# TritonDataCenter/containerpilot

Hardware: NVIDIA H100
Metric: events/sec through Bus.Publish (deliveries/s = 32-byte records landed in subscriber mailboxes) (higher is better)
Workload: dtype u8

## Files before the change

### containerpilot_b200/csrc/cpbus.cu

```cuda
#include "cpbus_kernels.cuh"

#include <algorithm>
#include <chrono>
#include <cstdio>
#include <cstdlib>
#include <cstring>
#include <deque>
#include <map>
#include <mutex>
#include <new>
#include <string>
#include <thread>
#include <unordered_map>
#include <vector>

using namespace cpbus_dev;

namespace {

thread_local char g_cuda_err[256] = "";

#define CK(call)                                                                                   \
  do {                                                                                             \
    cudaError_t e_ = (call);                                                                       \
// ... 561 lines not shown
  static bool done[64] = {};
  static std::mutex mu;
  std::lock_guard<std::mutex> g(mu);
  if (done[b->device & 63]) return CPBUS_OK;
  int rc;
  if ((rc = preload_round_fanouts<CPBUS_STORE_V4>()) || (rc = preload_round_fanouts<CPBUS_STORE_V8>()) ||
      (rc = preload_round_fanouts<CPBUS_STORE_BULK>()))
    return rc;
  cudaFuncAttributes a;
  CK(cudaFuncGetAttributes(&a, stream_round_decide_kernel));
  CK(cudaFuncGetAttributes(&a, stream_round_admit_kernel));
  CK(cudaFuncGetAttributes(&a, stream_round_agree_kernel));
  CK(cudaFuncGetAttributes(&a, consume_all_kernel));
  CK(cudaFuncGetAttributes(&a, digest_fold_kernel));
  CK(cudaFuncGetAttributes(&a, blockers_scan_kernel));
  CK(cudaFuncGetAttributes(&a, lagging_scan_kernel));
  done[b->device & 63] = true;
  return CPBUS_OK;
}

struct StreamArgs {
  const StreamHdr* hdr = nullptr; unsigned long long* ack = nullptr; unsigned long long seq = 0;
  const StreamHdr* next_hdr = nullptr;
  uint32_t off = 0; bool final = true;
  FollowRec* follow_rec = nullptr;
  bool follow_from_host = false;
  const RoundDev* round = nullptr;
};

struct LaunchOpts {
  int staged = 0;
  const cpbus_event* pf_src = nullptr;
  cpbus_event* pf_dst = nullptr;
  uint32_t pf_n = 0;
  bool batch_dep = false;
  bool account = false;
  const StreamArgs* stream = nullptr;
};

DevResultSlot* result_slot(const cpbus* b, unsigned long long seq) {
  return b->d_result + (size_t)(seq % kResultRing) * kResultSub;
}

void launched_to(cpbus* b, uint64_t w) {
  b->last_watermark = w;
  if (b->sparse) due_fire(b->due, b->h_timers, w, [](uint32_t, uint64_t, uint64_t) {});
}

int launch_fanout(cpbus* b, const cpbus_event* d_src, uint32_t n, uint64_t w, const LaunchOpts& o = {}) {
  const StreamArgs* sa = o.stream;
  if (b->n_next == 0 && !sa) return CPBUS_OK;
  if (n == 0 && b->n_timers == 0 && !sa) return CPBUS_OK;
  FanoutParams p{};
  p.batch = d_src; p.ring = b->d_ring; p.ctl = b->d_ctl; p.timers = b->d_timers; p.stats = b->d_stats; p.pow_table = b->d_pow; p.launch_seq = ++b->launch_seq;
  p.desc = b->d_desc + (p.launch_seq & 1) * ((fanout_desc_bytes(2048) + 255) & ~(size_t)255);
  p.desc_ready = b->d_desc_ready + (p.launch_seq & 1) * 16; p.w_now = w;
  p.result = result_slot(b, p.launch_seq); p.result_next = result_slot(b, p.launch_seq + 1);
  p.batch_local = b->d_batch_local; p.staged = (uint32_t)o.staged;
  p.err_word = b->d_err; p.acct = o.account ? b->d_acct : nullptr;
  p.pf_state = b->d_pf_state; p.pf_buf = b->d_pf_buf; p.pf_stride = b->B; p.spin_us = b->stream_spin_us;
  if (sa) {
    p.stream_hdr = sa->hdr; p.stream_ack = sa->ack; p.stream_seq = sa->seq; p.stream_next_hdr = sa->next_hdr;
    p.stream_off = sa->off; p.stream_final = sa->final ? 1u : 0u;
  }
  const bool follow = sa && sa->follow_rec, round = sa && sa->round;
  const int kind = round ? kLaunchRound : follow ? kLaunchFollow : kLaunchPlain;
  p.round = round ? sa->round : nullptr;
  if (follow) {
    p.follow_clock = b->d_follow_clock; p.follow_rec = sa->follow_rec; p.follow_window = max_window(b);
    p.follow_from_host = sa->follow_from_host ? 1u : 0u;
  }
  p.prefetch_src = o.pf_src; p.prefetch_dst = o.pf_dst; p.prefetch_n = o.pf_n;
  p.batch_dep = o.batch_dep ? 1u : 0u; p.n_ev = n;
  p.n_subs = b->n_next; p.ring_cap = b->R; p.K = b->K; p.sub_base = b->cfg.sub_id_base;
  p.use_digest = b->use_digest; p.lossless = b->lossless; p.timers_on = b->n_timers > 0 && b->K > 0;
  p.smem_cap = (n + 31u) & ~31u;
  const size_t hot_bytes = (size_t)b->n_next * (sizeof(SubCtl) + (p.timers_on ? b->K * sizeof(DevTimer) : 0));
  p.hints = b->hints >= 0 ? (uint32_t)b->hints : (hot_bytes <= (64u << 20) ? 1u : 0u);
  const uint32_t need = (b->n_next + kWarpsPerCta - 1) / kWarpsPerCta;
  uint32_t grid = b->cfg.grid_ctas ? std::max(1u, std::min(b->cfg.grid_ctas, need)) : 0u;
  int rc;
  const bool pairs_on = b->n_paired > 0 && b->d_pairs;
  p.pairs = pairs_on ? b->d_pairs : nullptr;
  size_t smem = fanout_smem_bytes(p.smem_cap) + (pairs_on ? kPairFilterBytes : 0);
  if (!pairs_on && !p.timers_on && b->n_filtered > 0) {
    if (b->order_dirty) { const int rc_order = rebuild_order(b); if (rc_order) return rc_order; }
    if (b->n_order) {
      const uint32_t scale = std::max(1u, (p.n_ev + 128u) / 256u);
      uint32_t spw = b->subs_per_warp ? std::min(32u, b->subs_per_warp)
                                      : std::max(4u, std::min(16u / scale, b->n_order / (20480u * scale)));
      p.order = b->d_order; p.n_order = b->n_order; p.spw = spw;
      const uint32_t warps = (b->n_order + spw - 1) / spw;
      grid = std::max(1u, (warps + kWarpsPerCta - 1) / kWarpsPerCta);
    }
  }
  if (pairs_on && !b->cfg.grid_ctas) {
    const uint32_t blocks = (b->n_next + 31u) / 32u;
    grid = std::max(1u, std::min((blocks + kWarpsPerCta - 1) / kWarpsPerCta, (uint32_t)b->sm_count * 16u));
  }
  if (!pairs_on && !p.order) {
    uint32_t spw = b->subs_per_warp;
    if (grid) spw = std::max(1u, (need + grid - 1) / grid);
    else if (!spw) {
      const uint32_t scale = std::max(1u, (p.n_ev + 128u) / 256u);
      const uint32_t cap = std::max(1u, 16u / scale);
      spw = std::max(1u, std::min(cap, (need + (uint32_t)b->sm_count * 7 * scale) / ((uint32_t)b->sm_count * 14 * scale)));
    }
    p.spw = spw;
    grid = std::max(1u, (need + spw - 1) / spw);
    const size_t off = fanout_stage_off(p.smem_cap);
    const size_t per_sub = sizeof(SubCtl) + (p.timers_on ? (size_t)b->K * sizeof(DevTimer) : 0);
    const size_t min_round = (size_t)kWarpsPerCta * per_sub;
    const size_t ctas = std::max<size_t>(1, std::min<size_t>(kCtasPerSm, b->smem_per_sm / (off + min_round + b->smem_reserved)));
    const size_t room = std::min<size_t>(kFanoutMaxSmem, b->smem_per_sm / ctas - b->smem_reserved) - off;
    p.stage_subs = std::max<uint32_t>(kWarpsPerCta, (uint32_t)std::min<size_t>((size_t)kWarpsPerCta * spw, room / per_sub) & ~7u);
    smem = off + p.stage_subs * per_sub;
  }
  const int variant = pairs_on ? (p.use_digest ? 7 : 6) : (p.timers_on ? 2 : 0) | (p.use_digest ? 1 : 0) | (p.order ? 4 : 0);
#define CPBUS_DISPATCH(ST)                                                                \
  switch (variant) {                                                                     \
    case 0: rc = launch_fanout_t<ST, false, false, false>(b, p, grid, smem, kind); break;      \
    case 1: rc = launch_fanout_t<ST, false, true, false>(b, p, grid, smem, kind); break;       \
    case 2: rc = launch_fanout_t<ST, true, false, false>(b, p, grid, smem, kind); break;       \
    case 3: rc = launch_fanout_t<ST, true, true, false>(b, p, grid, smem, kind); break;        \
    case 4: rc = launch_fanout_t<ST, false, false, true>(b, p, grid, smem, kind); break;       \
    case 5: rc = launch_fanout_t<ST, false, true, true>(b, p, grid, smem, kind); break;        \
    case 6: rc = launch_fanout_t<ST, true, false, false, true>(b, p, grid, smem, kind); break; \
    default: rc = launch_fanout_t<ST, true, true, false, true>(b, p, grid, smem, kind); break; \
  }
  switch (b->store) {
    case CPBUS_STORE_V4: CPBUS_DISPATCH(CPBUS_STORE_V4); break;
    case CPBUS_STORE_BULK: CPBUS_DISPATCH(CPBUS_STORE_BULK); break;
    default: CPBUS_DISPATCH(CPBUS_STORE_V8); break;
  }
#undef CPBUS_DISPATCH
  if (rc) return rc;
  b->st.kernel_launches++;
  if (!round) b->st.batches++;
  if (sa) return CPBUS_OK;
  launched_to(b, w);
  if (o.account && n) dbg_mark_device_batch(b, p.launch_seq);
  return CPBUS_OK;
}

void timer_table(cpbus* b) {
  b->h_timers.resize((size_t)b->N * b->K);
  if (b->sparse) b->due.init(b->h_timers.size());
}

int stage_batch(cpbus* b, uint32_t n, cpbus_event** d_dst) {
  const uint32_t slot = b->dev_slot;
  *d_dst = b->d_stage + (size_t)slot * b->B;
  if (slot % cpbus::kDevEpoch == 0) CK(cudaEventSynchronize(b->epoch_done[slot / cpbus::kDevEpoch]));
  if (n) {
    CK(cudaMemcpyAsync(*d_dst, b->h_batch[b->cur], (size_t)n * sizeof(cpbus_event), cudaMemcpyHostToDevice, b->copy_stream));
    CK(cudaEventRecord(b->h2d_done[b->cur], b->copy_stream));
  }
  return CPBUS_OK;
}

int retire_slot(cpbus* b) {
  const uint32_t slot = b->dev_slot;
  if (slot % cpbus::kDevEpoch == cpbus::kDevEpoch - 1) CK(cudaEventRecord(b->epoch_done[slot / cpbus::kDevEpoch], b->stream));
  b->dev_slot = (slot + 1) % cpbus::kDevSlots;
  return CPBUS_OK;
}

int await_copy(cpbus* b, cudaEvent_t copied) {
  const auto t_spin = std::chrono::steady_clock::now();
  do {
    const cudaError_t q = cudaEventQuery(copied);
    if (q == cudaSuccess) return CPBUS_OK;
    if (q != cudaErrorNotReady) { CK(q); }
  } while (std::chrono::steady_clock::now() - t_spin < std::chrono::microseconds(30));
  CK(cudaStreamWaitEvent(b->stream, copied, 0));
  return CPBUS_OK;
}

int next_buffer(cpbus* b) {
  b->cur = (b->cur + 1) % cpbus::kStage;
  CK(cudaEventSynchronize(b->h2d_done[b->cur]));
  return CPBUS_OK;
}

size_t sparse_max(const cpbus* b) { return std::max<size_t>(32, b->n_next / 1024); }
size_t sparse_max_deliveries(const cpbus* b) { return std::max<size_t>(1024, b->n_next / 256); }

int plan_room(cpbus* b, size_t bytes) {
  if (bytes <= b->plan_bytes_cap) { CK(cudaEventSynchronize(b->plan_done)); return CPBUS_OK; }
  CK(cudaStreamSynchronize(b->stream)); CK(cudaStreamSynchronize(b->copy_stream));
  cudaFree(b->d_plan); cudaFreeHost(b->h_plan);
  b->d_plan = nullptr; b->h_plan = nullptr; b->plan_bytes_cap = 0;
  const size_t cap = std::max<size_t>(bytes, 64 << 10);
// ... 2447 lines not shown
```

### containerpilot_b200/csrc/cpbus_fanout_body.cuh

```cuda
  constexpr bool STAGED = !ORDERED && !PAIRS;
  extern __shared__ __align__(128) unsigned char smem[];
  const uint32_t cap = p.smem_cap;
  cpbus_event* s_batch = reinterpret_cast<cpbus_event*>(smem);
  uint64_t* s_rhash = reinterpret_cast<uint64_t*>(smem + (size_t)cap * 32);
  uint2* s_meta = reinterpret_cast<uint2*>(smem + (size_t)cap * 40);
  uint64_t* s_q = reinterpret_cast<uint64_t*>(smem + (size_t)cap * 48);
  uint32_t* s_dsum = reinterpret_cast<uint32_t*>(s_q + cap + 2);
  uint32_t* s_present = s_dsum + 40;
  uint64_t* s_pow = s_q + cap + 2 + 20 + (PAIRS ? kPairFilterWords / 2 : 0);
  BatchSummary* s_sum = reinterpret_cast<BatchSummary*>(s_pow + cap + 66);
  uint32_t* s_tick = reinterpret_cast<uint32_t*>(s_sum + 1);
  const uint4* s_ctl4 = reinterpret_cast<const uint4*>(smem + fanout_stage_off(cap));
  const uint4* s_tim4 = s_ctl4 + 2u * p.stage_subs;

  const int tid = threadIdx.x, lane = tid & 31, warp = tid >> 5;
  uint32_t n = FOLLOW ? 0u : p.n_ev;
  uint64_t w_follow = 0;
  unsigned long long round_ack = 0;

  if (p.batch_dep) asm volatile("griddepcontrol.wait;" ::: "memory");
  const bool stream = p.staged == 2u;
  const uint32_t pf_slot = stream ? (uint32_t)(p.stream_seq % kStreamPrefetch) : 0u;
  uint32_t pos = ORDERED ? (blockIdx.x * kWarpsPerCta + warp) * p.spw : 0u;
  uint32_t my_ids = 0;
  if (ORDERED && pos + lane < min(pos + p.spw, p.n_order)) my_ids = __ldg(p.order + pos + lane);
  if (tid == 0) {
    mbar_init(&s_sum->mbar, 1); mbar_init(&s_sum->mbar_desc, 1); mbar_init(&s_sum->mbar_state, 1);
    s_sum->acc_deliv = 0; s_sum->acc_ticks = 0; s_sum->acc_dig_lo = 0; s_sum->acc_dig_hi = 0;
    s_sum->stream_local = (stream && !p.lossless && p.stream_off == 0 && __ldcg(p.pf_state + pf_slot) == p.stream_seq) ? 1u : 0u;
    s_sum->own_desc = blockIdx.x == 0 ? 1u : 0u; s_sum->abort_launch = 0;
  }
  __syncthreads();
  const bool stream_local = stream && s_sum->stream_local;
  const bool staged = FOLLOW || (p.staged && !stream_local);
  const cpbus_event* batch_src = stream_local ? p.pf_buf + (size_t)pf_slot * p.pf_stride : p.batch;
  if (tid == 0) {
    const uint32_t pow_bytes = ((cap + 65u) * 8u + 15u) & ~15u;
    const bool direct = n && !staged;
    mbar_expect_tx(&s_sum->mbar, (direct ? n * 32u : 0u) + pow_bytes);
    if (direct) bulk_g2s(s_batch, batch_src, n * 32u, &s_sum->mbar);
    bulk_g2s(s_pow, p.pow_table, pow_bytes, &s_sum->mbar);
  }

  const bool keep = p.hints & 1u;

  const uint32_t desc_bytes = 24u * cap + 16u + 160u + (PAIRS ? kPairFilterBytes : 0u);
  uint4* s_desc = reinterpret_cast<uint4*>(s_rhash);
  uint4* g_desc = reinterpret_cast<uint4*>(p.desc);
  constexpr unsigned long long kAbortBit = 1ull << 63;
  if (blockIdx.x != 0) {
    if (tid == 0) {
      unsigned long long seen = 0;
      if (!(p.hints & 2u)) {
        unsigned long long t0, t1;
        asm volatile("mov.u64 %0, %%globaltimer;" : "=l"(t0));
        const unsigned long long budget = stream ? 4000000000ull : 200000ull;
        do {
          asm volatile("ld.acquire.gpu.global.u64 %0, [%1];" : "=l"(seen) : "l"(p.desc_ready) : "memory");
          if ((seen & ~kAbortBit) >= p.launch_seq) break;
          asm volatile("mov.u64 %0, %%globaltimer;" : "=l"(t1));
        } while (t1 - t0 < budget);
      }
      if ((seen & ~kAbortBit) < p.launch_seq) s_sum->own_desc = 1u;
      else {
        const bool ab = (seen & kAbortBit) != 0;
        s_sum->abort_launch = ab ? 1u : 0u;
        asm volatile("fence.proxy.async;" ::: "memory");
        mbar_expect_tx(&s_sum->mbar_desc, desc_bytes);
        bulk_g2s(s_desc, g_desc, desc_bytes, &s_sum->mbar_desc);
        const uint32_t n_copy = FOLLOW ? (ab ? 0u : *reinterpret_cast<const volatile uint32_t*>(p.desc + 24u * cap + 16u + 4u * kFollowN)) : n;
        if (staged && n_copy && !ab) {
          mbar_wait(&s_sum->mbar, 0);
          mbar_expect_tx(&s_sum->mbar, n_copy * 32u);
          bulk_g2s(s_batch, p.batch_local, n_copy * 32u, &s_sum->mbar);
        }
      }
    }
    __syncthreads();
  }
  const bool own_desc = s_sum->own_desc != 0;
  const bool lead = blockIdx.x == 0;
  if (own_desc) {
    if (lead && tid < kResultSub * 4) reinterpret_cast<unsigned long long*>(p.result_next)[tid] = 0ull;
    if (tid < 40) s_dsum[tid] = 0;
    if constexpr (ROUND) {
      __syncthreads();
      if (tid == 0) {
        const volatile RoundDev* rd = p.round;
        if (!rd->go) s_sum->abort_launch = 1u;
        else {
          const unsigned long long w = rd->w;
          s_dsum[kFollowN] = rd->m; s_dsum[kFollowWLo] = (uint32_t)w; s_dsum[kFollowWHi] = (uint32_t)(w >> 32);
          s_dsum[kRoundSrc] = rd->src;
          if (lead && rd->final) round_ack = rd->q;
        }
// ... 183 lines not shown
  const uint32_t K = p.K, J = K ? 32u / K : 32u;
  const uint32_t tk_slot = lane / J, tk_j = lane % J;
  const bool timers_on = TIMERS && p.timers_on && K;
  const uint32_t wstride = gridDim.x * kWarpsPerCta;
  uint32_t pos_end = (aborted || !ORDERED) ? 0u : min(pos + p.spw, p.n_order);
  const uint32_t pos_step = ORDERED ? 1u : kWarpsPerCta;
  const uint32_t pos0 = pos;
  uint32_t s = ORDERED ? __shfl_sync(0xffffffffu, my_ids, 0) : pos;
  if (!p.batch_dep) asm volatile("griddepcontrol.wait;" ::: "memory");
  asm volatile("griddepcontrol.launch_dependents;");
  const uint32_t rng_first = blockIdx.x * kWarpsPerCta * p.spw, rng_end = min(rng_first + kWarpsPerCta * p.spw, p.n_subs);
  auto stage_round = [&](uint32_t first) {
    if (!STAGED || tid != 0 || aborted || first >= rng_end) return;
    const uint32_t rn = min(p.stage_subs, rng_end - first);
    asm volatile("fence.proxy.async.shared::cta;" ::: "memory");
    const uint32_t tim_bytes = timers_on ? rn * K * (uint32_t)sizeof(DevTimer) : 0u;
    mbar_expect_tx(&s_sum->mbar_state, rn * (uint32_t)sizeof(SubCtl) + tim_bytes);
    bulk_g2s_hint(const_cast<uint4*>(s_ctl4), p.ctl + first, rn * (uint32_t)sizeof(SubCtl), &s_sum->mbar_state, keep);
    if (tim_bytes) bulk_g2s_hint(const_cast<uint4*>(s_tim4), p.timers + (size_t)first * K, tim_bytes, &s_sum->mbar_state, keep);
  };
  uint4 ca = make_uint4(0, 0, 0, 0), cb = ca, ta = ca;
  if (ORDERED && pos < pos_end) ld_sector(p.ctl + s, ca, cb, keep);
  const uint32_t present = s_dsum[0];
  const bool has_unicast = s_dsum[1] != 0;
  bool bulk_pending = false;
  uint32_t tri_blk = blockIdx.x * kWarpsPerCta + warp, tri_base = 0, tri_live = 0;
  uint4 tri_a = make_uint4(0, 0, 0, 0), tri_b = tri_a;
  uint32_t rnd_first = rng_first, rnd_phase = 0;
  for (;;) {
  if constexpr (STAGED) {
    if (aborted || rnd_first >= rng_end) break;
    stage_round(rnd_first);
    mbar_wait(&s_sum->mbar_state, rnd_phase);
    rnd_phase ^= 1u;
    pos = rnd_first + warp; pos_end = rnd_first + min(p.stage_subs, rng_end - rnd_first);
  }
  if constexpr (PAIRS) {
    bool exhausted = aborted;
    while (!tri_live && !exhausted) {
      tri_base = tri_blk * 32u;
      if (tri_base >= p.n_subs) { exhausted = true; break; }
      tri_blk += wstride;
      const uint32_t sl = tri_base + lane;
      bool live = false;
      tri_a = make_uint4(0, 0, 0, 0); tri_b = tri_a;
      if (sl < p.n_subs) ld_sector(p.ctl + sl, tri_a, tri_b, keep);
      const uint32_t ml = tri_b.z;
      if (ml & kActiveBit) {
        live = has_unicast || (ml & present) != 0;
        if (!live && timers_on) {
          const uint32_t nsl = min((ml >> kTimerHintShift) & 0xFu, K);
          for (uint32_t t = 0; t < nsl && !live; t++) {
            uint4 h;
            ld_half(p.timers + (size_t)sl * K + t, h, keep);
            const uint64_t due = ((uint64_t)h.y << 32) | h.x;
            live = due != kTimerIdle && due <= (FOLLOW ? w_follow : p.w_now);
          }
        }
        if (!live && (ml & kPairBit)) {
          const uint4* row = reinterpret_cast<const uint4*>(p.pairs + (size_t)sl * CPBUS_MAX_PAIRS);
          for (uint32_t q = 0; q < CPBUS_MAX_PAIRS / 2 && !live; q++) {
            const uint4 v = __ldg(row + q);
            if (v.x >= 32u) break;
            uint32_t h = pair_key_hash(v.x, v.y);
            live = ((s_present[(h & 32767u) >> 5] >> (h & 31u)) & (s_present[((h >> 15) & 32767u) >> 5] >> ((h >> 15) & 31u)) & 1u) != 0;
            if (live || v.z >= 32u) { if (!live) break; continue; }
            h = pair_key_hash(v.z, v.w);
            live = ((s_present[(h & 32767u) >> 5] >> (h & 31u)) & (s_present[((h >> 15) & 32767u) >> 5] >> ((h >> 15) & 31u)) & 1u) != 0;
          }
        }
      }
      tri_live = __ballot_sync(0xffffffffu, live);
    }
    if (exhausted) break;
    const uint32_t jl = (uint32_t)__ffs(tri_live) - 1u;
    tri_live &= tri_live - 1u;
    pos = tri_base + jl; pos_end = pos + 1u; s = pos;
    ca = make_uint4(__shfl_sync(0xffffffffu, tri_a.x, jl), __shfl_sync(0xffffffffu, tri_a.y, jl), __shfl_sync(0xffffffffu, tri_a.z, jl), __shfl_sync(0xffffffffu, tri_a.w, jl));
    cb = make_uint4(__shfl_sync(0xffffffffu, tri_b.x, jl), __shfl_sync(0xffffffffu, tri_b.y, jl), __shfl_sync(0xffffffffu, tri_b.z, jl), __shfl_sync(0xffffffffu, tri_b.w, jl));
    if (timers_on && tk_slot < K) ld_half(p.timers + (size_t)s * K + tk_slot, ta, keep);
  }
  const uint32_t Rm = p.ring_cap - 1;
  const uint4* s4 = reinterpret_cast<const uint4*>(s_batch);
  const uint32_t scratch_words = max(32u, cap / 2u);
  uint32_t* my_tick = s_tick + warp * scratch_words;

  uint32_t run_mask = 0xffffffffu, run_k = 0;
  uint64_t run_sum = 0;
  for (; pos < pos_end; pos += pos_step) {
    const uint32_t si = pos - rnd_first;
    uint4 cur_a = ca, cur_b = cb;
    auto ctl_half = [&](uint32_t h) -> uint4 { return STAGED ? s_ctl4[2u * si + h] : (h ? cur_b : cur_a); };
    auto tim_half = [&](uint32_t h) -> uint4 {
      if (STAGED) return s_tim4[2u * (si * K + tk_slot) + h];
      if (!h) return ta;
      uint4 cold;
      ld_half(reinterpret_cast<const unsigned char*>(p.timers + (size_t)s * K + tk_slot) + 16, cold, keep);
      return cold;
    };
    if (STAGED) { cur_a = ctl_half(0); cur_b = ctl_half(1); }
    if (ORDERED) s = __shfl_sync(0xffffffffu, my_ids, (pos - pos0) & 31); else s = pos;
    if (ORDERED) {
      const uint32_t pn = pos + pos_step;
      if (pn < pos_end) ld_sector(p.ctl + __shfl_sync(0xffffffffu, my_ids, (pn - pos0) & 31), ca, cb, keep);
    }
    const uint32_t m = cur_b.z;
    if (!(m & kActiveBit)) continue;
    const uint64_t tail = ((uint64_t)cur_a.y << 32) | cur_a.x;
    cpbus_event* ring = p.ring + (size_t)s * p.ring_cap;
    const uint32_t gid = p.sub_base + s;
    const uint32_t nslots = timers_on ? min((m >> kTimerHintShift) & 0xFu, K) : 0u;
    const bool dense = !has_unicast && ((m & present) == present);

    uint32_t n_ticks = 0, tk_mask = 0, tk_rank = 0, tk_src = 0, tk_fired = 0;
    bool tk_valid = false; uint64_t tk_due = 0, tk_period = 0;
    if (nslots) {
      uint64_t tk_due0 = kTimerIdle;
      if (TIMERS && tk_slot < nslots) {
        const uint4 hot = tim_half(0);
        tk_due0 = ((uint64_t)hot.y << 32) | hot.x; tk_period = ((uint64_t)hot.w << 32) | hot.z;
      }
      const uint64_t step = (uint64_t)tk_j * tk_period;
      tk_due = tk_due0 + step;
      const bool wraps = __umul64hi(tk_j, tk_period) != 0 || tk_due < step || tk_due == kTimerIdle;
      tk_valid = tk_due0 != kTimerIdle && !wraps && tk_due <= (FOLLOW ? w_follow : p.w_now) && (tk_j == 0 || tk_period != 0);
      tk_mask = __ballot_sync(0xffffffffu, tk_valid);
      n_ticks = __popc(tk_mask);
      if (n_ticks) {

        if (J == 32 || (tk_mask >> J) == 0) tk_rank = tk_j;
        else {
#pragma unroll 1
          for (int t = 0; t < 32; t++) {
            if (!((tk_mask >> t) & 1u)) continue;
            const uint64_t od = shfl64(tk_due, t);
            const uint32_t os = __shfl_sync(0xffffffffu, tk_slot, t);
            tk_rank += (od < tk_due || (od == tk_due && os < tk_slot)) ? 1u : 0u;
          }
        }
      }
    }
    uint32_t tk_pos = 0;
    if (tk_valid) {
      uint32_t lo = 0, hi = n;
      while (lo < hi) {
        const uint32_t mid = (lo + hi) >> 1;
        if (ev_ts(mid) < tk_due) lo = mid + 1; else hi = mid;
      }
      tk_pos = lo;
    }

    bool pair_live = false;
    if (PAIRS && (m & kPairBit) && !dense) {
      uint2 pr = make_uint2(kPairNone, 0u);
      if (lane < CPBUS_MAX_PAIRS) pr = __ldg(p.pairs + (size_t)s * CPBUS_MAX_PAIRS + lane);
      bool hit = false;
      if (pr.x < 32u) {
        const uint32_t h = pair_key_hash(pr.x, pr.y);
        hit = ((s_present[(h & 32767u) >> 5] >> (h & 31u)) & (s_present[((h >> 15) & 32767u) >> 5] >> ((h >> 15) & 31u)) & 1u) != 0;
      }
      pair_live = __any_sync(0xffffffffu, hit);
    }
    if (PAIRS && !pair_live && !has_unicast && n_ticks == 0 && (m & present) == 0) continue;

    uint32_t k = 0;
    uint64_t dsum = 0;

    if (dense && n_ticks == 0) {
      if (STORE == CPBUS_STORE_BULK) {
        if (lane == 0 && n) {
          const uint32_t slot0 = (uint32_t)tail & Rm;
          const uint32_t first = min(n, p.ring_cap - slot0);
          bulk_s2g(ring + slot0, s_batch, first * 32u);
          if (n > first) bulk_s2g(ring, s_batch + first, (n - first) * 32u);
          asm volatile("cp.async.bulk.commit_group;" ::: "memory");
        }
        bulk_pending = true;
      } else if (STORE == CPBUS_STORE_V8) {
        for (uint32_t c0 = 0; c0 < n; c0 += 32)
          copy_record_pairs<PLANAR>(s4, hi_off, ring, (uint32_t)tail, Rm, c0 + lane, c0 + lane, c0 + lane < n);
      } else {
        for (uint32_t q = lane; q < 2 * n; q += 32) {
          const uint4 v = PLANAR ? s4[(q & 1u) * hi_off + (q >> 1)] : s4[q];
          st_v4(reinterpret_cast<unsigned char*>(ring + (((uint32_t)tail + (q >> 1)) & Rm)) + (q & 1u) * 16u, v);
        }
      }
      k = n;
      if (DIGEST) dsum = s_q[n];
    } else if (dense) {
      constexpr bool cold_early = !STAGED;
      if (cold_early && TIMERS && tk_slot < nslots) {
        const uint4 cold = tim_half(1);
        tk_src = cold.x; tk_fired = cold.y;
      }
      if (tk_valid) my_tick[tk_rank] = tk_pos;
      __syncwarp();
      k = n + n_ticks;
      const uint32_t T = (uint32_t)lane < n_ticks ? my_tick[lane] : 0xFFFFFFFFu;
      auto slot_of = [&](uint32_t c0) -> uint32_t {
        const uint32_t before = __popc(__ballot_sync(0xffffffffu, T <= c0));
        const bool in = T > c0 && T < c0 + 32u;
        const uint32_t n_in = __popc(__ballot_sync(0xffffffffu, in));
        const uint32_t i = c0 + lane;
        uint32_t out = i + before;
        if (n_in) {
          const uint32_t bits = __reduce_or_sync(0xffffffffu, in ? 1u << (T - c0) : 0u);
          if (__popc(bits) == n_in) out += __popc(bits & ((2u << lane) - 1u));
          else
            for (uint32_t t = before; t < n_ticks && my_tick[t] < c0 + 32u; t++) out += (my_tick[t] <= i) ? 1u : 0u;
        }
        return out;
      };
      uint32_t c0 = 0;
#pragma unroll 1
      for (; c0 + 64 <= n; c0 += 64) {
        const uint32_t o0 = slot_of(c0), o1 = slot_of(c0 + 32);
        copy_record_pairs<PLANAR>(s4, hi_off, ring, (uint32_t)tail, Rm, c0 + lane, o0, true);
        copy_record_pairs<PLANAR>(s4, hi_off, ring, (uint32_t)tail, Rm, c0 + 32 + lane, o1, true);
      }
#pragma unroll 1
      for (; c0 < n; c0 += 32) {
        const uint32_t out = slot_of(c0);
        copy_record_pairs<PLANAR>(s4, hi_off, ring, (uint32_t)tail, Rm, c0 + lane, out, c0 + lane < n);
      }
      if (!cold_early && TIMERS && tk_slot < nslots) {
        const uint4 cold = tim_half(1);
        tk_src = cold.x; tk_fired = cold.y;
      }
      if (tk_valid) {
        const uint32_t out = tk_pos + tk_rank;
        const uint64_t w0 = (uint64_t)tk_fired + tk_j, w1 = tk_due;
        const uint64_t w2 = (uint64_t)CPBUS_TIMER_EXPIRED | ((uint64_t)tk_src << 32);
        const uint64_t w3 = (uint64_t)gid | ((uint64_t)CPBUS_F_TICK << 32);
        const uint4 a = make_uint4((uint32_t)w0, (uint32_t)(w0 >> 32), (uint32_t)w1, (uint32_t)(w1 >> 32));
        const uint4 b = make_uint4((uint32_t)w2, (uint32_t)(w2 >> 32), (uint32_t)w3, (uint32_t)(w3 >> 32));
        st_v8(ring + (((uint32_t)tail + out) & Rm), a, b);
        if (DIGEST) {
          const uint32_t prev = tk_rank ? my_tick[tk_rank - 1] : 0u;
          dsum = (s_q[tk_pos] - s_q[prev]) * s_pow[n_ticks - tk_rank] + record_hash_words(w0, w1, w2, w3) * s_pow[k - 1 - out];
          if (tk_rank == n_ticks - 1) dsum += s_q[n] - s_q[tk_pos];
        }
      }
      if (DIGEST) dsum = warp_sum64(dsum);
      __syncwarp();
    } else if (!(PAIRS && pair_live) && !has_unicast && n_ticks == 0) {
      if constexpr (!TIMERS) {
        uint16_t* my_idx = reinterpret_cast<uint16_t*>(my_tick);
        const bool reuse = ORDERED && (m & CPBUS_MASK_ALL) == run_mask;
        if (!reuse) {
          uint32_t base = 0;
          const uint32_t nchunks = (n + 31) >> 5;
          for (uint32_t c0 = 0; c0 < nchunks; c0 += 4) {
            uint32_t cbit[4];
#pragma unroll
            for (uint32_t u = 0; u < 4; u++) {
              const uint32_t i = (c0 + u) * 32 + lane;
              cbit[u] = i < n ? s_meta[i].x : 0u;
            }
#pragma unroll
            for (uint32_t u = 0; u < 4; u++) {
              const bool match = (m & cbit[u]) != 0;
              const uint32_t w = __ballot_sync(0xffffffffu, match);
              if (match) my_idx[base + __popc(w & ((1u << lane) - 1u))] = (uint16_t)((c0 + u) * 32 + lane);
              base += __popc(w);
            }
          }
          run_k = base;
          __syncwarp();
        }
        k = run_k;
        uint64_t acc = 0;
        const uint64_t p32 = s_pow[32];
        const bool hashing = DIGEST && !reuse;
        uint32_t i0 = (uint32_t)lane < k ? my_idx[lane] : 0u, i1 = lane + 32u < k ? my_idx[lane + 32] : 0u;
        for (uint32_t o0 = 0; o0 < k; o0 += 64) {
          const uint32_t o = o0 + lane;
          const bool v0 = o < k, v1 = o + 32 < k;
          const uint32_t n0 = o + 64 < k ? my_idx[o + 64] : 0u, n1 = o + 96 < k ? my_idx[o + 96] : 0u;
          copy_record_pairs<PLANAR>(s4, hi_off, ring, (uint32_t)tail, Rm, i0, o, v0);
          copy_record_pairs<PLANAR>(s4, hi_off, ring, (uint32_t)tail, Rm, i1, o + 32, v1);
          if (hashing) {
            if (v0) acc = acc * p32 + s_rhash[i0];
            if (v1) acc = acc * p32 + s_rhash[i1];
          }
          i0 = n0; i1 = n1;
        }
        if (DIGEST) {
          if (reuse) dsum = run_sum;
          else {
            const uint32_t cnt = k > (uint32_t)lane ? (k - lane + 31u) / 32u : 0u;
            dsum = cnt ? acc * s_pow[k - 1 - (lane + 32u * (cnt - 1u))] : 0ull;
            dsum = warp_sum64(dsum);
            if (ORDERED) run_sum = dsum;
          }
        }
        if (ORDERED) run_mask = m & CPBUS_MASK_ALL;
        __syncwarp();
      } else {
        uint32_t kk = ((m >> lane) & 1u) ? s_dsum[2 + lane] : 0u;
        kk = __reduce_add_sync(0xffffffffu, kk);
        k = kk;
        uint32_t base = 0;
        const uint32_t nchunks = (n + 31) >> 5;
        for (uint32_t c = 0; c < nchunks; c++) {
          const uint32_t i = c * 32 + lane;
          const bool match = i < n && (m & s_meta[i].x) != 0;
          const uint32_t w = __ballot_sync(0xffffffffu, match);
          const uint32_t out = base + __popc(w & ((1u << lane) - 1u));
          if (DIGEST && match) dsum += s_rhash[i] * s_pow[k - 1 - out];
          copy_record_pairs<PLANAR>(s4, hi_off, ring, (uint32_t)tail, Rm, i, out, match);
          base += __popc(w);
        }
        if (DIGEST) dsum = warp_sum64(dsum);
      }
    } else {
      const uint32_t nchunks = (n + 31) >> 5;
      uint2 my_pair = make_uint2(kPairNone, 0u);
      uint32_t n_pairs = 0, pair_codes = 0;
      if (PAIRS && pair_live) {
        if (lane < CPBUS_MAX_PAIRS) my_pair = __ldg(p.pairs + (size_t)s * CPBUS_MAX_PAIRS + lane);
        const bool used = my_pair.x < 32u;
        n_pairs = __popc(__ballot_sync(0xffffffffu, used));
        pair_codes = __reduce_or_sync(0xffffffffu, used ? (1u << my_pair.x) : 0u);
      }
// ... 189 lines not shown
```

### containerpilot_b200/csrc/cpbus_kernels.cuh

```cuda
#pragma once
#include <cstdint>
#include <cuda_runtime.h>

#include "../../include/cpbus.h"

namespace cpbus_dev {

constexpr int kWarpsPerCta = 8;
constexpr int kThreads = kWarpsPerCta * 32;
constexpr int kCtasPerSm = 4;
constexpr uint32_t kActiveBit = 0x80000000u;
constexpr int kTimerHintShift = 24;
constexpr uint32_t kPairBit = 0x10000000u;
constexpr uint32_t kPairNone = 0xFFFFFFFFu;
constexpr uint32_t kCodeOutOfRange = CPBUS_N_CODES;
static_assert(kCodeOutOfRange < (uint32_t)kTimerHintShift,"the out-of-range bit must lie between the code mask and the mask word's bookkeeping bits");
constexpr uint32_t kPairFilterWords = 1024;
constexpr uint32_t kPairFilterBytes = kPairFilterWords * 4;
__host__ __device__ inline uint32_t pair_key_hash(uint32_t code, uint32_t source_id) {
  uint32_t x = (source_id ^ (code << 27)) * 0x9E3779B1u;
  x ^= x >> 15; x *= 0x85EBCA77u; x ^= x >> 13;
  return x;
}
constexpr uint64_t kDigestP = 0x9E3779B97F4A7C15ull;
// ... 124 lines not shown
  cpbus_event* prefetch_dst;
  uint32_t prefetch_n;
  uint32_t batch_dep;
  const uint32_t* order;
  uint32_t n_order, spw;
  uint32_t stage_subs;
  uint64_t w_now;
  uint32_t n_ev, n_subs, ring_cap, K, sub_base;
  uint32_t use_digest, lossless, timers_on;
  uint32_t smem_cap;
  uint32_t hints;
  const uint2* pairs;
  const StreamHdr* stream_hdr;
  unsigned long long* stream_ack;
  unsigned long long stream_seq;
  const StreamHdr* stream_next_hdr;
  uint32_t stream_off;
  uint32_t stream_final;
  unsigned long long* pf_state;
  cpbus_event* pf_buf;
  uint32_t pf_stride;
  uint32_t spin_us;
  unsigned int* err_word;
  DevPubAcct* acct;
  unsigned long long* follow_clock;
  FollowRec* follow_rec;
  uint64_t follow_window;
  uint32_t follow_from_host;
  const RoundDev* round;
};

__host__ __device__ inline uint64_t record_hash_words(uint64_t w0, uint64_t w1, uint64_t w2, uint64_t w3) {
  const uint64_t K0 = 0x9E3779B97F4A7C15ull, K1 = 0xBF58476D1CE4E5B9ull,
                 K2 = 0x94D049BB133111EBull, K3 = 0xD6E8FEB86659FD93ull,
                 K4 = 0xA0761D6478BD642Full;
  uint64_t x = (w0 + K4) * K0; x ^= x >> 32;
  x = (x + w1) * K1; x ^= x >> 32;
  x = (x + w2) * K2; x ^= x >> 32;
  x = (x + w3) * K3; x ^= x >> 29;
  return x;
}

__host__ __device__ inline uint64_t pow_p(uint32_t e) {
  uint64_t r = 1, b = kDigestP;
  while (e) { if (e & 1u) r *= b; b *= b; e >>= 1; }
  return r;
}

#ifdef __CUDACC__
__device__ __forceinline__ uint32_t smem_u32(const void* p) { return (uint32_t)__cvta_generic_to_shared(p); }
__device__ __forceinline__ uint64_t shfl64(uint64_t v, int src) {
  uint32_t lo = __shfl_sync(0xffffffffu, (uint32_t)v, src);
  uint32_t hi = __shfl_sync(0xffffffffu, (uint32_t)(v >> 32), src);
  return ((uint64_t)hi << 32) | lo;
}
__device__ __forceinline__ uint64_t warp_sum64(uint64_t v) {
#pragma unroll
  for (int o = 16; o > 0; o >>= 1) {
    uint32_t lo = __shfl_xor_sync(0xffffffffu, (uint32_t)v, o);
    uint32_t hi = __shfl_xor_sync(0xffffffffu, (uint32_t)(v >> 32), o);
    v += ((uint64_t)hi << 32) | lo;
  }
  return v;
}
__device__ __forceinline__ void st_v4(void* dst, const uint4& a) {
  asm volatile("st.global.v4.b32 [%0], {%1,%2,%3,%4};" ::"l"(dst), "r"(a.x), "r"(a.y), "r"(a.z), "r"(a.w) : "memory");
}
__device__ __forceinline__ void st_v8(void* dst, const uint4& a, const uint4& b) {
  st_v4(dst, a);
  st_v4(reinterpret_cast<unsigned char*>(dst) + 16, b);
}
template <bool PL>
__device__ __forceinline__ void copy_record_pairs(const uint4* s4, uint32_t hi, cpbus_event* ring, uint32_t tail, uint32_t Rm,
                                                  uint32_t i, uint32_t out, bool valid) {
  const uint32_t h = threadIdx.x & 1u, ev = (threadIdx.x & 31u) & ~1u;
  const uint32_t pi = __shfl_xor_sync(0xffffffffu, i, 1), po = __shfl_xor_sync(0xffffffffu, out, 1);
  const uint32_t vm = __ballot_sync(0xffffffffu, valid);
  const uint32_t ie = h ? pi : i, oe = h ? po : out, io = h ? i : pi, oo = h ? out : po;
  if ((vm >> ev) & 1u)
    st_v4(reinterpret_cast<unsigned char*>(ring + ((tail + oe) & Rm)) + 16u * h, PL ? s4[h * hi + ie] : s4[2u * ie + h]);
  if ((vm >> (ev + 1u)) & 1u)
    st_v4(reinterpret_cast<unsigned char*>(ring + ((tail + oo) & Rm)) + 16u * h, PL ? s4[h * hi + io] : s4[2u * io + h]);
}
__device__ __forceinline__ uint64_t keep_policy() {
  uint64_t pol;
  asm volatile("createpolicy.fractional.L2::evict_last.b64 %0, 1.0;" : "=l"(pol));
  return pol;
}
__device__ __forceinline__ void ld_half(const void* src, uint4& a, bool hinted);
__device__ __forceinline__ void st_half(void* dst, const uint4& a, bool hinted);
__device__ __forceinline__ void ld_sector(const void* src, uint4& a, uint4& b, bool hinted) {
  ld_half(src, a, hinted);
  ld_half(reinterpret_cast<const unsigned char*>(src) + 16, b, hinted);
}
__device__ __forceinline__ void st_sector(void* dst, const uint4& a, const uint4& b, bool hinted) {
  st_half(dst, a, hinted);
  st_half(reinterpret_cast<unsigned char*>(dst) + 16, b, hinted);
}
__device__ __forceinline__ void ld_half(const void* src, uint4& a, bool hinted) {
  const uint64_t pol = hinted ? keep_policy() : 0ull;
  if (hinted)
    asm volatile("ld.global.L2::cache_hint.v4.b32 {%0,%1,%2,%3}, [%4], %5;" : "=r"(a.x), "=r"(a.y), "=r"(a.z), "=r"(a.w) : "l"(src), "l"(pol));
  else
    asm volatile("ld.global.v4.b32 {%0,%1,%2,%3}, [%4];" : "=r"(a.x), "=r"(a.y), "=r"(a.z), "=r"(a.w) : "l"(src));
}
__device__ __forceinline__ void st_half(void* dst, const uint4& a, bool hinted) {
  const uint64_t pol = hinted ? keep_policy() : 0ull;
  if (hinted)
    asm volatile("st.global.L2::cache_hint.v4.b32 [%0], {%1,%2,%3,%4}, %5;" ::"l"(dst), "r"(a.x), "r"(a.y), "r"(a.z), "r"(a.w), "l"(pol) : "memory");
  else st_v4(dst, a);
}
__device__ __forceinline__ void bulk_g2s(void* sdst, const void* gsrc, uint32_t bytes, uint64_t* mbar) {
  asm volatile("cp.async.bulk.shared::cluster.global.mbarrier::complete_tx::bytes [%0], [%1], %2, [%3];" ::"r"(
                   smem_u32(sdst)),
               "l"(gsrc), "r"(bytes), "r"(smem_u32(mbar))
               : "memory");
}
__device__ __forceinline__ void bulk_g2s_hint(void* sdst, const void* gsrc, uint32_t bytes, uint64_t* mbar, bool hinted) {
  if (!hinted) { bulk_g2s(sdst, gsrc, bytes, mbar); return; }
  asm volatile("cp.async.bulk.shared::cluster.global.mbarrier::complete_tx::bytes.L2::cache_hint [%0], [%1], %2, [%3], %4;" ::"r"(
                   smem_u32(sdst)),
               "l"(gsrc), "r"(bytes), "r"(smem_u32(mbar)), "l"(keep_policy())
               : "memory");
}
__device__ __forceinline__ void bulk_s2g(void* gdst, const void* ssrc, uint32_t bytes) {
  asm volatile("cp.async.bulk.global.shared::cta.bulk_group [%0], [%1], %2;" ::"l"(gdst), "r"(smem_u32(ssrc)),
               "r"(bytes)
               : "memory");
}
__device__ __forceinline__ void mbar_init(uint64_t* mbar, uint32_t count) {
  asm volatile("mbarrier.init.shared::cta.b64 [%0], %1;" ::"r"(smem_u32(mbar)), "r"(count));
  asm volatile("fence.mbarrier_init.release.cluster;" ::: "memory");
}
__device__ __forceinline__ void mbar_expect_tx(uint64_t* mbar, uint32_t bytes) {
  asm volatile("mbarrier.arrive.expect_tx.shared::cta.b64 _, [%0], %1;" ::"r"(smem_u32(mbar)), "r"(bytes) : "memory");
}
__device__ __forceinline__ void mbar_wait(uint64_t* mbar, uint32_t parity) {
  asm volatile(
      "{\n\t.reg .pred p;\n\t"
      "CPBUS_WAIT:\n\t"
      "mbarrier.try_wait.parity.shared::cta.b64 p, [%0], %1;\n\t"
      "@p bra CPBUS_DONE;\n\t"
      "bra CPBUS_WAIT;\n\t"
      "CPBUS_DONE:\n\t}" ::"r"(smem_u32(mbar)),
      "r"(parity)
      : "memory");
}

struct BatchSummary {
  uint64_t mbar;
  uint64_t mbar_desc;
  uint64_t mbar_state;
  uint32_t acc_deliv, acc_ticks, acc_pad[2];
  uint32_t acc_dig_lo, acc_dig_hi;
  uint32_t stream_local;
  uint32_t own_desc;
  uint32_t abort_launch;
  uint32_t pf_ok;
  uint64_t red[kWarpsPerCta];
};

__host__ __device__ inline size_t fanout_desc_bytes(uint32_t cap) { return (size_t)24 * cap + 16 + 160 + kPairFilterBytes; }

__host__ __device__ inline size_t fanout_smem_bytes(uint32_t cap) {
  const size_t scratch = (cap / 2u > 32u ? cap / 2u : 32u) * sizeof(uint32_t);
  return (size_t)cap * 56 + 16 + 160 + (size_t)(cap + 66) * 8 + sizeof(BatchSummary) + kWarpsPerCta * scratch + 128;
}
__host__ __device__ inline size_t fanout_stage_off(uint32_t cap) { return (fanout_smem_bytes(cap) + 127) & ~(size_t)127; }

template <int STORE, bool TIMERS, bool DIGEST, bool ORDERED, bool PAIRS = false>
__global__ void __launch_bounds__(kThreads, kCtasPerSm) fanout_kernel(const FanoutParams p) {
  constexpr bool FOLLOW = false, ROUND = false;
#include "cpbus_fanout_body.cuh"
}
template <int STORE, bool TIMERS, bool DIGEST, bool ORDERED, bool PAIRS = false>
__global__ void __launch_bounds__(kThreads, kCtasPerSm) fanout_follow_kernel(const FanoutParams p) {
  constexpr bool FOLLOW = true, ROUND = false;
#include "cpbus_fanout_body.cuh"
}
template <int STORE, bool TIMERS, bool DIGEST, bool ORDERED, bool PAIRS = false>
__global__ void __launch_bounds__(kThreads, kCtasPerSm) fanout_round_kernel(const FanoutParams p) {
  constexpr bool FOLLOW = true, ROUND = true;
#include "cpbus_fanout_body.cuh"
}

__device__ __forceinline__ void admit_body(const cpbus_event* batch, uint32_t n_ev, uint64_t w_now, const SubCtl* ctl,
                                           const DevTimer* timers, uint32_t n_subs, uint32_t ring_cap, uint32_t K,
                                           uint32_t sub_base, uint32_t timers_on, DevStats* stats, const uint2* pairs) {
  __shared__ uint32_t hist[32];
  __shared__ uint32_t s_uni;
  __shared__ unsigned long long s_max;
  if (threadIdx.x < 32) hist[threadIdx.x] = 0;
  if (threadIdx.x == 0) { s_uni = 0; s_max = 0; }
  __syncthreads();
  for (uint32_t i = threadIdx.x; i < n_ev; i += blockDim.x) {
    const uint32_t code = batch[i].code, target = batch[i].target;
    if (target == CPBUS_TARGET_ALL) { if (code < 32) atomicAdd(&hist[code], 1u); }
    else atomicAdd(&s_uni, 1u);
  }
  __syncthreads();
  const uint32_t s = blockIdx.x * blockDim.x + threadIdx.x;
  SubCtl c{};
  if (s < n_subs) c = ctl[s];
  const uint32_t m = c.mask;
  if (s < n_subs && (m & kActiveBit)) {
    uint64_t k = 0;
    for (uint32_t cc = 0; cc < CPBUS_N_CODES; cc++) if ((m >> cc) & 1u) k += hist[cc];
    if (pairs && (m & kPairBit)) {
      const uint2* my = pairs + (size_t)s * CPBUS_MAX_PAIRS;
      for (uint32_t i = 0; i < n_ev; i++) {
        const uint32_t code = batch[i].code;
        if (batch[i].target != CPBUS_TARGET_ALL || code >= CPBUS_N_CODES || ((m >> code) & 1u)) continue;
        const uint32_t src = batch[i].source_id;
        for (uint32_t j = 0; j < CPBUS_MAX_PAIRS; j++) {
          const uint2 pr = my[j];
          if (pr.x == kPairNone) break;
          if (pr.x == code && pr.y == src) { k++; break; }
        }
      }
    }
    if (s_uni) {
      const uint32_t gid = sub_base + s;
      for (uint32_t i = 0; i < n_ev; i++) if (batch[i].target == gid) k++;
    }
    const uint32_t nslots = timers_on ? min((m >> kTimerHintShift) & 0xFu, K) : 0u;
    const uint64_t w_due = min(w_now, kTimerIdle - 1);
    for (uint32_t t = 0; t < nslots; t++) {
      const DevTimer tm = timers[(size_t)s * K + t];
      if (tm.next_due != kTimerIdle && tm.next_due <= w_due)
        k += tm.period ? (w_due - tm.next_due) / tm.period + 1u : 1u;
    }
    const unsigned long long used = c.tail - c.head + k;
    if (used > ring_cap) {
      atomicAdd(&stats->admit_overflow, 1ull);
      const unsigned long long room = ring_cap - min((unsigned long long)ring_cap, c.tail - c.head);
      const uint32_t gid = sub_base + s;
      unsigned long long taken = 0;
      uint32_t prefix = 0;
      for (uint32_t i = 0; i < n_ev; i++) {
        const cpbus_event e = batch[i];
        unsigned long long tks = 0;
        for (uint32_t t = 0; t < nslots; t++) {
          const DevTimer tm = timers[(size_t)s * K + t];
          const uint64_t ts = min(e.ts_ns, kTimerIdle - 1);
          if (tm.next_due != kTimerIdle && tm.next_due <= ts) tks += tm.period ? (ts - tm.next_due) / tm.period + 1u : 1u;
        }
        bool want;
        if (e.target == CPBUS_TARGET_ALL) {
          want = e.code < CPBUS_N_CODES && ((m >> e.code) & 1u);
          if (!want && pairs && (m & kPairBit)) {
            const uint2* my = pairs + (size_t)s * CPBUS_MAX_PAIRS;
// ... 717 lines not shown
```

Baseline: 93.14 billion.

## Stage timer tick records in shared scratch and merge into dense ring copy

Adds a dense-path branch for non-pair kernels where each warp writes its fired timer tick records into per-warp shared scratch. One merged pass then copies batch events and tick records into the subscriber ring with paired 16-byte stores, using ballot-based ranking to interleave them. To make room for the records, the per-warp scratch floor grows when timers are enabled, which raises shared memory per CTA and may reduce staging room or occupancy. The digest contribution of the ticks is computed inline.

```diff
diff --git a/containerpilot_b200/csrc/cpbus.cu b/containerpilot_b200/csrc/cpbus.cu
--- a/containerpilot_b200/csrc/cpbus.cu
+++ b/containerpilot_b200/csrc/cpbus.cu
@@ -667,7 +667,8 @@
   int rc;
   const bool pairs_on = b->n_paired > 0 && b->d_pairs;
   p.pairs = pairs_on ? b->d_pairs : nullptr;
-  size_t smem = fanout_smem_bytes(p.smem_cap) + (pairs_on ? kPairFilterBytes : 0);
+  const bool tick_records = !pairs_on && p.timers_on;
+  size_t smem = fanout_smem_bytes(p.smem_cap, tick_records) + (pairs_on ? kPairFilterBytes : 0);
   if (!pairs_on && !p.timers_on && b->n_filtered > 0) {
     if (b->order_dirty) { const int rc_order = rebuild_order(b); if (rc_order) return rc_order; }
     if (b->n_order) {
@@ -693,7 +694,7 @@
     }
     p.spw = spw;
     grid = std::max(1u, (need + spw - 1) / spw);
-    const size_t off = fanout_stage_off(p.smem_cap);
+    const size_t off = fanout_stage_off(p.smem_cap, tick_records);
     const size_t per_sub = sizeof(SubCtl) + (p.timers_on ? (size_t)b->K * sizeof(DevTimer) : 0);
     const size_t min_round = (size_t)kWarpsPerCta * per_sub;
     const size_t ctas = std::max<size_t>(1, std::min<size_t>(kCtasPerSm, b->smem_per_sm / (off + min_round + b->smem_reserved)));
diff --git a/containerpilot_b200/csrc/cpbus_fanout_body.cuh b/containerpilot_b200/csrc/cpbus_fanout_body.cuh
--- a/containerpilot_b200/csrc/cpbus_fanout_body.cuh
+++ b/containerpilot_b200/csrc/cpbus_fanout_body.cuh
@@ -10,7 +10,7 @@
   uint64_t* s_pow = s_q + cap + 2 + 20 + (PAIRS ? kPairFilterWords / 2 : 0);
   BatchSummary* s_sum = reinterpret_cast<BatchSummary*>(s_pow + cap + 66);
   uint32_t* s_tick = reinterpret_cast<uint32_t*>(s_sum + 1);
-  const uint4* s_ctl4 = reinterpret_cast<const uint4*>(smem + fanout_stage_off(cap));
+  const uint4* s_ctl4 = reinterpret_cast<const uint4*>(smem + fanout_stage_off(cap, TIMERS && !PAIRS));
   const uint4* s_tim4 = s_ctl4 + 2u * p.stage_subs;
 
   const int tid = threadIdx.x, lane = tid & 31, warp = tid >> 5;
@@ -360,7 +360,7 @@
   }
   const uint32_t Rm = p.ring_cap - 1;
   const uint4* s4 = reinterpret_cast<const uint4*>(s_batch);
-  const uint32_t scratch_words = max(32u, cap / 2u);
+  const uint32_t scratch_words = max(fanout_scratch_floor(TIMERS && !PAIRS), cap / 2u);
   uint32_t* my_tick = s_tick + warp * scratch_words;
 
   uint32_t run_mask = 0xffffffffu, run_k = 0;
@@ -465,6 +465,43 @@
       }
       k = n;
       if (DIGEST) dsum = s_q[n];
+    } else if (dense && !PAIRS) {
+      if (TIMERS && tk_slot < nslots) {
+        const uint4 cold = tim_half(1);
+        tk_src = cold.x; tk_fired = cold.y;
+      }
+      k = n + n_ticks;
+      const uint32_t tk_out = tk_pos + tk_rank;
+      uint4* rec = reinterpret_cast<uint4*>(my_tick);
+      if (tk_valid) {
+        const uint64_t w0 = (uint64_t)tk_fired + tk_j, w1 = tk_due;
+        const uint64_t w2 = (uint64_t)CPBUS_TIMER_EXPIRED | ((uint64_t)tk_src << 32);
+        const uint64_t w3 = (uint64_t)gid | ((uint64_t)CPBUS_F_TICK << 32);
+        rec[2u * tk_rank] = make_uint4((uint32_t)w0, (uint32_t)(w0 >> 32), (uint32_t)w1, (uint32_t)(w1 >> 32));
+        rec[2u * tk_rank + 1u] = make_uint4((uint32_t)w2, (uint32_t)(w2 >> 32), (uint32_t)w3, (uint32_t)(w3 >> 32));
+        if (DIGEST) {
+          dsum = s_q[tk_pos] * (s_pow[n_ticks - tk_rank] - s_pow[n_ticks - tk_rank - 1]) +
+                 record_hash_words(w0, w1, w2, w3) * s_pow[k - 1 - tk_out];
+          if (tk_rank == 0) dsum += s_q[n];
+        }
+      }
+      __syncwarp();
+      const uint32_t rec0 = (uint32_t)(rec - s4);
+      const uint32_t lt = (1u << lane) - 1u;
+      uint32_t before = 0;
+#pragma unroll 1
+      for (uint32_t o0 = 0u - ((uint32_t)tail & 3u); (int)o0 < (int)k; o0 += 32) {
+        const uint32_t d = tk_out - o0;
+        const uint32_t bits = __reduce_or_sync(0xffffffffu, tk_valid && d < 32u ? 1u << d : 0u);
+        const uint32_t r = before + __popc(bits & lt);
+        const uint32_t i = o0 + lane - r;
+        const bool tick = (bits >> lane) & 1u;
+        const uint32_t s0 = tick ? rec0 + 2u * r : PLANAR ? i : 2u * i;
+        copy_slot_pairs(s4, ring, (uint32_t)tail, Rm, o0, k, s0, tick ? s0 + 1u : PLANAR ? s0 + hi_off : s0 + 1u);
+        before += __popc(bits);
+      }
+      if (DIGEST) dsum = warp_sum64(dsum);
+      __syncwarp();
     } else if (dense) {
       constexpr bool cold_early = !STAGED;
       if (cold_early && TIMERS && tk_slot < nslots) {
diff --git a/containerpilot_b200/csrc/cpbus_kernels.cuh b/containerpilot_b200/csrc/cpbus_kernels.cuh
--- a/containerpilot_b200/csrc/cpbus_kernels.cuh
+++ b/containerpilot_b200/csrc/cpbus_kernels.cuh
@@ -230,6 +230,13 @@
   if ((vm >> (ev + 1u)) & 1u)
     st_v4(reinterpret_cast<unsigned char*>(ring + ((tail + oo) & Rm)) + 16u * h, PL ? s4[h * hi + io] : s4[2u * io + h]);
 }
+__device__ __forceinline__ void copy_slot_pairs(const uint4* s4, cpbus_event* ring, uint32_t tail, uint32_t Rm, uint32_t o0, uint32_t k,
+                                                uint32_t s0, uint32_t s1) {
+  const uint32_t h = threadIdx.x & 1u, oe = o0 + ((threadIdx.x & 31u) & ~1u);
+  const uint32_t own = h ? s1 : s0, other = __shfl_xor_sync(0xffffffffu, h ? s0 : s1, 1);
+  if (oe < k) st_v4(reinterpret_cast<unsigned char*>(ring + ((tail + oe) & Rm)) + 16u * h, s4[h ? other : own]);
+  if (oe + 1u < k) st_v4(reinterpret_cast<unsigned char*>(ring + ((tail + oe + 1u) & Rm)) + 16u * h, s4[h ? own : other]);
+}
 __device__ __forceinline__ uint64_t keep_policy() {
   uint64_t pol;
   asm volatile("createpolicy.fractional.L2::evict_last.b64 %0, 1.0;" : "=l"(pol));
@@ -310,11 +317,13 @@
 
 __host__ __device__ inline size_t fanout_desc_bytes(uint32_t cap) { return (size_t)24 * cap + 16 + 160 + kPairFilterBytes; }
 
-__host__ __device__ inline size_t fanout_smem_bytes(uint32_t cap) {
-  const size_t scratch = (cap / 2u > 32u ? cap / 2u : 32u) * sizeof(uint32_t);
+__host__ __device__ inline constexpr uint32_t fanout_scratch_floor(bool tick_records) { return tick_records ? 256u : 32u; }
+__host__ __device__ inline size_t fanout_smem_bytes(uint32_t cap, bool tick_records) {
+  const uint32_t floor = fanout_scratch_floor(tick_records);
+  const size_t scratch = (cap / 2u > floor ? cap / 2u : floor) * sizeof(uint32_t);
   return (size_t)cap * 56 + 16 + 160 + (size_t)(cap + 66) * 8 + sizeof(BatchSummary) + kWarpsPerCta * scratch + 128;
 }
-__host__ __device__ inline size_t fanout_stage_off(uint32_t cap) { return (fanout_smem_bytes(cap) + 127) & ~(size_t)127; }
+__host__ __device__ inline size_t fanout_stage_off(uint32_t cap, bool tick_records) { return (fanout_smem_bytes(cap, tick_records) + 127) & ~(size_t)127; }
 
 template <int STORE, bool TIMERS, bool DIGEST, bool ORDERED, bool PAIRS = false>
 __global__ void __launch_bounds__(kThreads, kCtasPerSm) fanout_kernel(const FanoutParams p) {
```

Measured after the change: 95.45 billion, median of 6. +2.5%, better.

## Write dense fan-out output by destination slot with inline tick records

Applied to the files above, without the earlier changes.

Restructures the dense mailbox copy so each lane walks output slots rather than source records. Each lane computes whether its slot holds a source event or a timer tick by shuffling packed tick positions. Tick records are now built and stored inside the same coalesced pair-store pass instead of in a separate scattered store afterwards. This removes the per-chunk ballot/reduce slot computation and the extra tick stores, at the cost of per-slot tick scans and extra shuffles when ticks are present. The branch is now excluded for PAIRS, and the tick word index is derived from K via a bit trick that assumes K is a power of two.

```diff
diff --git a/containerpilot_b200/csrc/cpbus_fanout_body.cuh b/containerpilot_b200/csrc/cpbus_fanout_body.cuh
--- a/containerpilot_b200/csrc/cpbus_fanout_body.cuh
+++ b/containerpilot_b200/csrc/cpbus_fanout_body.cuh
@@ -465,59 +465,36 @@
       }
       k = n;
       if (DIGEST) dsum = s_q[n];
-    } else if (dense) {
-      constexpr bool cold_early = !STAGED;
-      if (cold_early && TIMERS && tk_slot < nslots) {
+    } else if (!PAIRS && dense) {
+      if (TIMERS && tk_slot < nslots) {
         const uint4 cold = tim_half(1);
         tk_src = cold.x; tk_fired = cold.y;
       }
-      if (tk_valid) my_tick[tk_rank] = tk_pos;
+      if (tk_valid) my_tick[tk_rank] = tk_pos | ((uint32_t)lane << 16);
       __syncwarp();
       k = n + n_ticks;
-      const uint32_t T = (uint32_t)lane < n_ticks ? my_tick[lane] : 0xFFFFFFFFu;
-      auto slot_of = [&](uint32_t c0) -> uint32_t {
-        const uint32_t before = __popc(__ballot_sync(0xffffffffu, T <= c0));
-        const bool in = T > c0 && T < c0 + 32u;
-        const uint32_t n_in = __popc(__ballot_sync(0xffffffffu, in));
-        const uint32_t i = c0 + lane;
-        uint32_t out = i + before;
-        if (n_in) {
-          const uint32_t bits = __reduce_or_sync(0xffffffffu, in ? 1u << (T - c0) : 0u);
-          if (__popc(bits) == n_in) out += __popc(bits & ((2u << lane) - 1u));
-          else
-            for (uint32_t t = before; t < n_ticks && my_tick[t] < c0 + 32u; t++) out += (my_tick[t] <= i) ? 1u : 0u;
-        }
-        return out;
-      };
-      uint32_t c0 = 0;
+      const uint32_t TS = (uint32_t)lane < n_ticks ? my_tick[lane] + lane : 0xFFFFFFFFu;
+      uint32_t before = 0;
 #pragma unroll 1
-      for (; c0 + 64 <= n; c0 += 64) {
-        const uint32_t o0 = slot_of(c0), o1 = slot_of(c0 + 32);
-        copy_record_pairs<PLANAR>(s4, hi_off, ring, (uint32_t)tail, Rm, c0 + lane, o0, true);
-        copy_record_pairs<PLANAR>(s4, hi_off, ring, (uint32_t)tail, Rm, c0 + 32 + lane, o1, true);
-      }
-#pragma unroll 1
-      for (; c0 < n; c0 += 32) {
-        const uint32_t out = slot_of(c0);
-        copy_record_pairs<PLANAR>(s4, hi_off, ring, (uint32_t)tail, Rm, c0 + lane, out, c0 + lane < n);
-      }
-      if (!cold_early && TIMERS && tk_slot < nslots) {
-        const uint4 cold = tim_half(1);
-        tk_src = cold.x; tk_fired = cold.y;
-      }
-      if (tk_valid) {
+      for (uint32_t o0 = 0; o0 < k; o0 += 32) {
+        const uint32_t o = o0 + lane;
+        const uint32_t upto = __popc(__ballot_sync(0xffffffffu, (TS & 0xFFFFu) < o0 + 32u));
+        uint32_t src = o - before;
+        for (uint32_t r = before; r < upto; r++) {
+          const uint32_t t = __shfl_sync(0xffffffffu, TS, r);
+          if ((t & 0xFFFFu) < o) src--;
+          else if ((t & 0xFFFFu) == o) src = kTickSrc | (t >> 16);
+        }
+        copy_output_pairs<PLANAR>(s4, hi_off, ring, (uint32_t)tail, Rm, o0, k, src, upto != before, K, tk_fired, tk_due, tk_src, gid);
+        before = upto;
+      }
+      if (DIGEST && tk_valid) {
         const uint32_t out = tk_pos + tk_rank;
-        const uint64_t w0 = (uint64_t)tk_fired + tk_j, w1 = tk_due;
         const uint64_t w2 = (uint64_t)CPBUS_TIMER_EXPIRED | ((uint64_t)tk_src << 32);
         const uint64_t w3 = (uint64_t)gid | ((uint64_t)CPBUS_F_TICK << 32);
-        const uint4 a = make_uint4((uint32_t)w0, (uint32_t)(w0 >> 32), (uint32_t)w1, (uint32_t)(w1 >> 32));
-        const uint4 b = make_uint4((uint32_t)w2, (uint32_t)(w2 >> 32), (uint32_t)w3, (uint32_t)(w3 >> 32));
-        st_v8(ring + (((uint32_t)tail + out) & Rm), a, b);
-        if (DIGEST) {
-          const uint32_t prev = tk_rank ? my_tick[tk_rank - 1] : 0u;
-          dsum = (s_q[tk_pos] - s_q[prev]) * s_pow[n_ticks - tk_rank] + record_hash_words(w0, w1, w2, w3) * s_pow[k - 1 - out];
-          if (tk_rank == n_ticks - 1) dsum += s_q[n] - s_q[tk_pos];
-        }
+        const uint32_t prev = tk_rank ? my_tick[tk_rank - 1] & 0xFFFFu : 0u;
+        dsum = (s_q[tk_pos] - s_q[prev]) * s_pow[n_ticks - tk_rank] + record_hash_words((uint64_t)tk_fired + tk_j, tk_due, w2, w3) * s_pow[k - 1 - out];
+        if (tk_rank == n_ticks - 1) dsum += s_q[n] - s_q[tk_pos];
       }
       if (DIGEST) dsum = warp_sum64(dsum);
       __syncwarp();
diff --git a/containerpilot_b200/csrc/cpbus_kernels.cuh b/containerpilot_b200/csrc/cpbus_kernels.cuh
--- a/containerpilot_b200/csrc/cpbus_kernels.cuh
+++ b/containerpilot_b200/csrc/cpbus_kernels.cuh
@@ -230,6 +230,28 @@
   if ((vm >> (ev + 1u)) & 1u)
     st_v4(reinterpret_cast<unsigned char*>(ring + ((tail + oo) & Rm)) + 16u * h, PL ? s4[h * hi + io] : s4[2u * io + h]);
 }
+constexpr uint32_t kTickSrc = 0x80000000u;
+template <bool PL>
+__device__ __forceinline__ void copy_output_pairs(const uint4* s4, uint32_t hi, cpbus_event* ring, uint32_t tail, uint32_t Rm,
+                                                  uint32_t o0, uint32_t k, uint32_t src, bool ticks, uint32_t K,
+                                                  uint32_t tk_fired, uint64_t tk_due, uint32_t tk_src, uint32_t gid) {
+  const uint32_t lane = threadIdx.x & 31u, h = lane & 1u, ev = lane & ~1u;
+  const uint32_t ps = __shfl_xor_sync(0xffffffffu, src, 1);
+#pragma unroll
+  for (uint32_t q = 0; q < 2; q++) {
+    const uint32_t c = (h == q) ? src : ps, o = o0 + ev + q;
+    uint4 v = make_uint4(0, 0, 0, 0);
+    if (!(c & kTickSrc) && o < k) v = PL ? s4[h * hi + c] : s4[2u * c + h];
+    if (ticks) {
+      const uint32_t t = c & 31u;
+      const uint64_t w0 = (uint64_t)__shfl_sync(0xffffffffu, tk_fired, t) + (t & (0x1Fu >> (__ffs(K) - 1)));
+      const uint32_t d0 = __shfl_sync(0xffffffffu, (uint32_t)tk_due, t), d1 = __shfl_sync(0xffffffffu, (uint32_t)(tk_due >> 32), t);
+      const uint32_t sr = __shfl_sync(0xffffffffu, tk_src, t);
+      if (c & kTickSrc) v = h ? make_uint4(CPBUS_TIMER_EXPIRED, sr, gid, CPBUS_F_TICK) : make_uint4((uint32_t)w0, (uint32_t)(w0 >> 32), d0, d1);
+    }
+    if (o < k) st_v4(reinterpret_cast<unsigned char*>(ring + ((tail + o) & Rm)) + 16u * h, v);
+  }
+}
 __device__ __forceinline__ uint64_t keep_policy() {
   uint64_t pol;
   asm volatile("createpolicy.fractional.L2::evict_last.b64 %0, 1.0;" : "=l"(pol));
```

After: 93.20 billion before, 95.32 billion after, median of 6. 2.3% higher.
